# nyuolab/OmniBioTE

Hardware: AMD Instinct MI355X
Metric: MLM train tokens/sec, small (8L/1024d) ctx=1024 at 1/2/4/8 MI355X (higher is better)
Workload: dtype bf16

## Files before the change

omnibiote_amd/csrc/elementwise.hip:

```cpp
#include "common.h"
#include <stdlib.h>

namespace {

template <bool INVERSE>
__global__ __launch_bounds__(256) void rope_kernel(bf16* __restrict__ qkv, const float* __restrict__ cos_t,
                                                    const float* __restrict__ sin_t, int64_t rows, int64_t T, int C, int hs) {
    const int chunks_per_row = 2 * C / 8;
    const int64_t total = rows * chunks_per_row;
    for (int64_t i = (int64_t)blockIdx.x * blockDim.x + threadIdx.x; i < total; i += (int64_t)gridDim.x * blockDim.x) {
        const int64_t row = i / chunks_per_row;
        const int col = (int)(i % chunks_per_row) * 8;
        const int d = col % hs;
        const int64_t t = row % T;
        bf16* ptr = qkv + row * 3 * C + col;
        const bf16x8 v = *reinterpret_cast<const bf16x8*>(ptr);
        const f32x4 c = *reinterpret_cast<const f32x4*>(cos_t + t * (hs / 2) + d / 2);
        const f32x4 s = *reinterpret_cast<const f32x4*>(sin_t + t * (hs / 2) + d / 2);
        bf16x8 o;
#pragma unroll
        for (int j = 0; j < 4; ++j) {
            const float xe = bf2f(v[2 * j]), xo = bf2f(v[2 * j + 1]);
            const float sj = INVERSE ? -s[j] : s[j];
            o[2 * j] = f2bf(xe * c[j] - xo * sj);
            o[2 * j + 1] = f2bf(xe * sj + xo * c[j]);
        }
        *reinterpret_cast<bf16x8*>(ptr) = o;
    }
}

__device__ __forceinline__ int64_t clamp_tok(int64_t tok, int64_t vocab) { return tok < 0 ? 0 : (tok >= vocab ? vocab - 1 : tok); }

__global__ __launch_bounds__(256) void embed_fwd_kernel(const int64_t* __restrict__ idx, const bf16* __restrict__ wte,
                                                         bf16* __restrict__ out, int64_t rows, int cols, int64_t vocab, DropCfg dc) {
    const int cpr = cols / 8;
    const int64_t total = rows * cpr;
    for (int64_t i = (int64_t)blockIdx.x * blockDim.x + threadIdx.x; i < total; i += (int64_t)gridDim.x * blockDim.x) {
        const int64_t r = i / cpr;
        const int c = (int)(i % cpr) * 8;
        const int64_t tok = clamp_tok(idx[r], vocab);
        bf16x8 v = *reinterpret_cast<const bf16x8*>(wte + tok * cols + c);
        if (dc.thresh16) {
            const uint32_t rk = drop_rowkey((uint64_t)r, dc);
#pragma unroll
            for (int jj = 0; jj < 4; ++jj) {
                const uint32_t bits = drop_pair_bits(rk, (uint32_t)(c >> 1) + jj);
#pragma unroll
                for (int e = 0; e < 2; ++e) v[2 * jj + e] = drop_keep_bits(bits, (uint32_t)e, dc) ? f2bf(bf2f(v[2 * jj + e]) * dc.scale) : f2bf(0.f);
            }
        }
        *reinterpret_cast<bf16x8*>(out + r * cols + c) = v;
    }
}

__global__ __launch_bounds__(256) void dropout_kernel(const bf16* in, bf16* out, int64_t n8, int64_t cols, DropCfg dc) {
    for (int64_t i = (int64_t)blockIdx.x * blockDim.x + threadIdx.x; i < n8; i += (int64_t)gridDim.x * blockDim.x) {
        bf16x8 v = reinterpret_cast<const bf16x8*>(in)[i];
        const int64_t row = (i * 8) / cols;
        const uint32_t c = (uint32_t)((i * 8) - row * cols);
        const uint32_t rk = drop_rowkey((uint64_t)row, dc);
        for (int jj = 0; jj < 4; ++jj) {
            const uint32_t bits = drop_pair_bits(rk, (c >> 1) + jj);
#pragma unroll
            for (int e = 0; e < 2; ++e) v[2 * jj + e] = drop_keep_bits(bits, (uint32_t)e, dc) ? f2bf(bf2f(v[2 * jj + e]) * dc.scale) : f2bf(0.f);
        }
        reinterpret_cast<bf16x8*>(out)[i] = v;
    }
}

constexpr int EMB_CHUNK = 32;

template <bool ACC>
__device__ __forceinline__ void embed_store_row(bf16* dst, const float (&acc)[8]) {
    bf16x8 o;
#pragma unroll
    for (int j = 0; j < 8; ++j) o[j] = f2bf(acc[j]);
    if (ACC) {
        const bf16x8 old = *reinterpret_cast<const bf16x8*>(dst);
#pragma unroll
        for (int j = 0; j < 8; ++j) o[j] = f2bf(bf2f(old[j]) + bf2f(o[j]));
    }
    *reinterpret_cast<bf16x8*>(dst) = o;
}
template <bool ACC>
__device__ __forceinline__ void embed_store_row(float* dst, const float (&acc)[8]) {
    f32x4 lo = f32x4{acc[0], acc[1], acc[2], acc[3]}, hi = f32x4{acc[4], acc[5], acc[6], acc[7]};
    if (ACC) {
        lo += *reinterpret_cast<const f32x4*>(dst);
        hi += *reinterpret_cast<const f32x4*>(dst + 4);
    }
    *reinterpret_cast<f32x4*>(dst) = lo;
    *reinterpret_cast<f32x4*>(dst + 4) = hi;
}

template <bool ACC, class DST = bf16>
__global__ __launch_bounds__(128) void embed_bwd_chunk_kernel(const int64_t* __restrict__ idx, const int32_t* __restrict__ order,
                                                               const bf16* __restrict__ dout, DST* __restrict__ dwte,
                                                               float* __restrict__ slab, int64_t rows, int cols, int64_t vocab, DropCfg dc) {
    __shared__ int32_t s_row[EMB_CHUNK];
    __shared__ int64_t s_tok[EMB_CHUNK + 2];
    const int64_t c = blockIdx.x;
    const int64_t p0 = c * EMB_CHUNK;
    const int n = (int)((rows - p0) < EMB_CHUNK ? (rows - p0) : EMB_CHUNK);
    if (threadIdx.x < n) {
        const int32_t r = order[p0 + threadIdx.x];
        s_row[threadIdx.x] = r;
        s_tok[threadIdx.x + 1] = clamp_tok(idx[r], vocab);
    }
    if (threadIdx.x == 64) s_tok[0] = p0 > 0 ? clamp_tok(idx[order[p0 - 1]], vocab) : -1;
    if (threadIdx.x == 65) s_tok[n + 1] = (p0 + n < rows) ? clamp_tok(idx[order[p0 + n]], vocab) : -1;
    __syncthreads();
    const bool left_open = s_tok[0] == s_tok[1];
    const bool right_open = s_tok[n + 1] == s_tok[n];
    for (int col = threadIdx.x * 8; col < cols; col += 128 * 8) {
        float acc[8];
#pragma unroll
        for (int j = 0; j < 8; ++j) acc[j] = 0.f;
        int seg_start = 0;
        for (int i = 0; i < n; ++i) {
            const bf16x8 v = *reinterpret_cast<const bf16x8*>(dout + (int64_t)s_row[i] * cols + col);
            if (dc.thresh16) {
                const uint32_t rk = drop_rowkey((uint64_t)s_row[i], dc);
                for (int jj = 0; jj < 4; ++jj) {
                    const uint32_t bits = drop_pair_bits(rk, (uint32_t)(col >> 1) + jj);
#pragma unroll
                    for (int e = 0; e < 2; ++e)
                        if (drop_keep_bits(bits, (uint32_t)e, dc)) acc[2 * jj + e] += bf2f(f2bf(bf2f(v[2 * jj + e]) * dc.scale));
                }
            } else {
#pragma unroll
                for (int j = 0; j < 8; ++j) acc[j] += bf2f(v[j]);
            }
            const bool seg_end = (i == n - 1) || (s_tok[i + 2] != s_tok[i + 1]);
            if (seg_end) {
                const bool is_first = seg_start == 0, is_last = i == n - 1;
                if ((is_first && left_open) || (is_last && right_open)) {
                    float* dst = slab + ((c * 2 + (is_first ? 0 : 1)) * cols + col);
                    *reinterpret_cast<f32x4*>(dst) = f32x4{acc[0], acc[1], acc[2], acc[3]};
                    *reinterpret_cast<f32x4*>(dst + 4) = f32x4{acc[4], acc[5], acc[6], acc[7]};
                } else {
                    embed_store_row<ACC>(dwte + s_tok[i + 1] * cols + col, acc);
                }
#pragma unroll
                for (int j = 0; j < 8; ++j) acc[j] = 0.f;
                seg_start = i + 1;
            }
        }
    }
}

template <bool ACC, class DST = bf16>
__global__ __launch_bounds__(128) void embed_bwd_span_kernel(const int64_t* __restrict__ idx, const int32_t* __restrict__ order,
                                                              DST* __restrict__ dwte, const float* __restrict__ slab,
                                                              int64_t rows, int cols, int64_t nchunks, int64_t vocab) {
    const int64_t c = blockIdx.x;
    const int64_t p0 = c * EMB_CHUNK;
    const int64_t p1 = (p0 + EMB_CHUNK < rows) ? p0 + EMB_CHUNK : rows;
    const int64_t first = clamp_tok(idx[order[p0]], vocab), last = clamp_tok(idx[order[p1 - 1]], vocab);
    const bool single = first == last;
    const bool left_open = p0 > 0 && clamp_tok(idx[order[p0 - 1]], vocab) == first;
    const bool right_open = p1 < rows && clamp_tok(idx[order[p1]], vocab) == last;
    if (!right_open || (single && left_open)) return;
    const int slot0 = single ? 0 : 1;
    for (int col = threadIdx.x * 8; col < cols; col += 128 * 8) {
        float acc[8];
        const float* src = slab + ((c * 2 + slot0) * cols + col);
#pragma unroll
        for (int j = 0; j < 8; ++j) acc[j] = src[j];
        for (int64_t cc = c + 1; cc < nchunks; ++cc) {
            const int64_t q0 = cc * EMB_CHUNK;
            const int64_t q1 = (q0 + EMB_CHUNK < rows) ? q0 + EMB_CHUNK : rows;
            if (clamp_tok(idx[order[q0]], vocab) != last) break;
            const float* s2 = slab + ((cc * 2) * cols + col);
#pragma unroll
            for (int j = 0; j < 8; ++j) acc[j] += s2[j];
            if (clamp_tok(idx[order[q1 - 1]], vocab) != last) break;
        }
        embed_store_row<ACC>(dwte + last * cols + col, acc);
    }
}

__global__ __launch_bounds__(256) void acc32_add_kernel(float* __restrict__ acc32, const bf16* __restrict__ src, bf16* __restrict__ out,
                                                         int64_t n8, int mode) {
    for (int64_t i = (int64_t)blockIdx.x * 256 + threadIdx.x; i < n8; i += (int64_t)gridDim.x * 256) {
        float v[8];
        if (src) {
            const bf16x8 sv = *reinterpret_cast<const bf16x8*>(src + i * 8);
#pragma unroll
            for (int j = 0; j < 8; ++j) v[j] = bf2f(sv[j]);
        } else {
#pragma unroll
            for (int j = 0; j < 8; ++j) v[j] = 0.f;
        }
        if (mode != OBTE_ACC32_FIRST) {
            const f32x4 lo = *reinterpret_cast<const f32x4*>(acc32 + i * 8), hi = *reinterpret_cast<const f32x4*>(acc32 + i * 8 + 4);
#pragma unroll
            for (int j = 0; j < 4; ++j) { v[j] += lo[j]; v[4 + j] += hi[j]; }
        }
        if (src || mode == OBTE_ACC32_FIRST) {
            *reinterpret_cast<f32x4*>(acc32 + i * 8) = f32x4{v[0], v[1], v[2], v[3]};
            *reinterpret_cast<f32x4*>(acc32 + i * 8 + 4) = f32x4{v[4], v[5], v[6], v[7]};
        }
        if (mode == OBTE_ACC32_LAST) {
            bf16x8 o;
#pragma unroll
            for (int j = 0; j < 8; ++j) o[j] = f2bf(v[j]);
            *reinterpret_cast<bf16x8*>(out + i * 8) = o;
        }
    }
}

__global__ __launch_bounds__(256) void masked_ce_kernel(const bf16* __restrict__ logits, const int64_t* __restrict__ target,
                                                         const uint8_t* __restrict__ mlm_mask, const uint8_t* __restrict__ prev_mask,
                                                         const float* __restrict__ grad_scale, float row_scale,
                                                         float* __restrict__ row_loss, bf16* __restrict__ dlogits, int64_t vocab,
                                                         const int64_t* __restrict__ row_index, const float* __restrict__ row_scale_vec) {
    __shared__ float red[8];
    const int64_t r = blockIdx.x;
    const int64_t src = row_index ? row_index[r] : r;
    const int lane = threadIdx.x & 63, wave = threadIdx.x >> 6;
    bf16* drow = dlogits + r * vocab;
    if (!row_index && mlm_mask && !mlm_mask[r]) {
        if (threadIdx.x == 0 && row_loss) row_loss[r] = 0.f;
        if (prev_mask && !prev_mask[r]) return;
        const bf16x8 z = {};
        for (int64_t c = (int64_t)threadIdx.x * 8; c < vocab; c += 256 * 8) *reinterpret_cast<bf16x8*>(drow + c) = z;
        return;
    }
    const bf16* lrow = logits + src * vocab;
    float m = -INFINITY, l = 0.f;
    for (int64_t c = (int64_t)threadIdx.x * 8; c < vocab; c += 256 * 8) {
        const bf16x8 v = *reinterpret_cast<const bf16x8*>(lrow + c);
// ... 475 lines not shown
    const int lane = threadIdx.x & 63;
    const uint32_t rk = drop_rowkey((uint64_t)rows[i], cfg);
    for (int c = lane * 8; c < cols; c += 512) {
        bf16x8 v = *reinterpret_cast<const bf16x8*>(in + i * cols + c);
        bf16x8 a = {};
        if (aux) a = *reinterpret_cast<const bf16x8*>(aux + i * cols + c);
#pragma unroll
        for (int jj = 0; jj < 4; ++jj) {
            const uint32_t bits = drop_pair_bits(rk, ((uint32_t)c >> 1) + jj);
#pragma unroll
            for (int e = 0; e < 2; ++e) {
                const int j = 2 * jj + e;
                const float t = drop_keep_bits(bits, (uint32_t)e, cfg) ? bf2f(f2bf(bf2f(v[j]) * cfg.scale)) : 0.f;
                v[j] = aux ? f2bf(bf2f(a[j]) + t) : f2bf(t);
            }
        }
        *reinterpret_cast<bf16x8*>(out + i * cols + c) = v;
    }
}

extern "C" int obte_dropout_bf16(const obte_bf16* in, obte_bf16* out, int64_t n, int64_t cols, float p, uint64_t seed, int32_t site,
                                 obte_stream s) {
    OBTE_REQUIRE_ALIGNED("obte_dropout_bf16", in, "in", 16);
    OBTE_REQUIRE_ALIGNED("obte_dropout_bf16", out, "out", 16);
    OBTE_REQUIRE(in && out && n > 0 && n % 8 == 0, "obte_dropout_bf16: null pointer or n not a positive multiple of 8");
    OBTE_REQUIRE(cols > 0 && cols % 8 == 0 && n % cols == 0 && cols < (1ll << 32), "obte_dropout_bf16: cols must be a multiple of 8 that divides n");
    if (check_p("obte_dropout_bf16", p)) return OBTE_EINVAL;
    hipLaunchKernelGGL(dropout_kernel, dim3(stream_grid(n / 8, 256)), dim3(256), 0, (hipStream_t)s, (const bf16*)in, (bf16*)out, n / 8,
                       cols, make_drop(p, seed, (uint32_t)site));
    OBTE_CHECK_LAUNCH("obte_dropout_bf16");
    return OBTE_OK;
}

extern "C" int64_t obte_embedding_bwd_ws_bytes(int64_t rows, int cols) {
    return cdiv64(rows, EMB_CHUNK) * 2 * (int64_t)cols * (int64_t)sizeof(float);
}

extern "C" int obte_embedding_bwd_dropout(const int64_t* idx, const int32_t* order, const obte_bf16* dout, obte_bf16* dwte,
                                          void* ws, int64_t rows, int cols, int64_t vocab, int accumulate, float p, uint64_t seed,
                                          obte_stream s) {
    OBTE_REQUIRE(idx && order && dout && dwte && ws, "obte_embedding_bwd: null pointer");
    OBTE_REQUIRE_ALIGNED("obte_embedding_bwd", dout, "dout", 16);
    OBTE_REQUIRE_ALIGNED("obte_embedding_bwd", dwte, "dwte", 16);
    OBTE_REQUIRE_ALIGNED("obte_embedding_bwd", ws, "ws", 16);
    if (check_p("obte_embedding_bwd", p)) return OBTE_EINVAL;
    const DropCfg dc = make_drop(p, seed, OBTE_SITE_EMBED);
    OBTE_REQUIRE(rows > 0 && cols > 0 && cols % 8 == 0 && vocab > 0, "obte_embedding_bwd: bad shape");
    OBTE_REQUIRE(rows < (1ll << 31), "obte_embedding_bwd: too many rows");
    hipStream_t st = (hipStream_t)s;
    if (!accumulate && hipMemsetAsync(dwte, 0, (size_t)vocab * cols * sizeof(obte_bf16), st) != hipSuccess) {
        obte_set_error("obte_embedding_bwd: memset failed");
        return OBTE_ELAUNCH;
    }
    const int64_t nchunks = cdiv64(rows, EMB_CHUNK);
    if (accumulate)
        hipLaunchKernelGGL(embed_bwd_chunk_kernel<true>, dim3((unsigned)nchunks), dim3(128), 0, st, idx, order, (const bf16*)dout,
                           (bf16*)dwte, (float*)ws, rows, cols, vocab, dc);
    else
        hipLaunchKernelGGL(embed_bwd_chunk_kernel<false>, dim3((unsigned)nchunks), dim3(128), 0, st, idx, order, (const bf16*)dout,
                           (bf16*)dwte, (float*)ws, rows, cols, vocab, dc);
    OBTE_CHECK_LAUNCH("obte_embedding_bwd(chunk)");
    if (accumulate)
        hipLaunchKernelGGL(embed_bwd_span_kernel<true>, dim3((unsigned)nchunks), dim3(128), 0, st, idx, order, (bf16*)dwte,
                           (const float*)ws, rows, cols, nchunks, vocab);
    else
        hipLaunchKernelGGL(embed_bwd_span_kernel<false>, dim3((unsigned)nchunks), dim3(128), 0, st, idx, order, (bf16*)dwte,
                           (const float*)ws, rows, cols, nchunks, vocab);
    OBTE_CHECK_LAUNCH("obte_embedding_bwd(span)");
    return OBTE_OK;
}

extern "C" int obte_acc32_add_bf16(float* acc32, const obte_bf16* src, obte_bf16* out, int64_t n, int mode, obte_stream s) {
    OBTE_REQUIRE_ALIGNED("obte_acc32_add_bf16", acc32, "acc32", 16);
    OBTE_REQUIRE_ALIGNED("obte_acc32_add_bf16", src, "src", 16);
    OBTE_REQUIRE_ALIGNED("obte_acc32_add_bf16", out, "out", 16);
    OBTE_REQUIRE(acc32 && n > 0 && n % 8 == 0, "obte_acc32_add_bf16: null buffer or n not a positive multiple of 8");
    OBTE_REQUIRE(mode >= OBTE_ACC32_FIRST && mode <= OBTE_ACC32_LAST && (mode != OBTE_ACC32_LAST || out), "obte_acc32_add_bf16: bad mode, or LAST without out");
    if (!src && mode == OBTE_ACC32_MORE) return OBTE_OK;
    hipLaunchKernelGGL(acc32_add_kernel, dim3(stream_grid(n / 8, 256)), dim3(256), 0, (hipStream_t)s, acc32, (const bf16*)src, (bf16*)out, n / 8, mode);
    OBTE_CHECK_LAUNCH("obte_acc32_add_bf16");
    return OBTE_OK;
}

extern "C" int obte_embedding_bwd_acc32(const int64_t* idx, const int32_t* order, const obte_bf16* dout, float* acc32, obte_bf16* dwte,
                                        void* ws, int64_t rows, int cols, int64_t vocab, int mode, float p, uint64_t seed, obte_stream s) {
    OBTE_REQUIRE(idx && order && dout && acc32 && ws, "obte_embedding_bwd_acc32: null pointer");
    OBTE_REQUIRE_ALIGNED("obte_embedding_bwd_acc32", dout, "dout", 16);
    OBTE_REQUIRE_ALIGNED("obte_embedding_bwd_acc32", acc32, "acc32", 16);
    OBTE_REQUIRE_ALIGNED("obte_embedding_bwd_acc32", dwte, "dwte", 16);
    OBTE_REQUIRE_ALIGNED("obte_embedding_bwd_acc32", ws, "ws", 16);
    OBTE_REQUIRE(mode >= OBTE_ACC32_FIRST && mode <= OBTE_ACC32_LAST && (mode != OBTE_ACC32_LAST || dwte), "obte_embedding_bwd_acc32: bad mode, or LAST without dwte");
    if (check_p("obte_embedding_bwd_acc32", p)) return OBTE_EINVAL;
    const DropCfg dc = make_drop(p, seed, OBTE_SITE_EMBED);
    OBTE_REQUIRE(rows > 0 && cols > 0 && cols % 8 == 0 && vocab > 0, "obte_embedding_bwd_acc32: bad shape");
    OBTE_REQUIRE(rows < (1ll << 31), "obte_embedding_bwd_acc32: too many rows");
    hipStream_t st = (hipStream_t)s;
    const bool first = mode == OBTE_ACC32_FIRST;
    if (first && hipMemsetAsync(acc32, 0, (size_t)vocab * cols * sizeof(float), st) != hipSuccess) {
        obte_set_error("obte_embedding_bwd_acc32: memset failed");
        return OBTE_ELAUNCH;
    }
    const int64_t nchunks = cdiv64(rows, EMB_CHUNK);
    if (first)
        hipLaunchKernelGGL((embed_bwd_chunk_kernel<false, float>), dim3((unsigned)nchunks), dim3(128), 0, st, idx, order, (const bf16*)dout, acc32, (float*)ws,
                           rows, cols, vocab, dc);
    else
        hipLaunchKernelGGL((embed_bwd_chunk_kernel<true, float>), dim3((unsigned)nchunks), dim3(128), 0, st, idx, order, (const bf16*)dout, acc32, (float*)ws,
                           rows, cols, vocab, dc);
    OBTE_CHECK_LAUNCH("obte_embedding_bwd_acc32(chunk)");
    if (first)
        hipLaunchKernelGGL((embed_bwd_span_kernel<false, float>), dim3((unsigned)nchunks), dim3(128), 0, st, idx, order, acc32, (const float*)ws, rows, cols,
                           nchunks, vocab);
    else
        hipLaunchKernelGGL((embed_bwd_span_kernel<true, float>), dim3((unsigned)nchunks), dim3(128), 0, st, idx, order, acc32, (const float*)ws, rows, cols,
                           nchunks, vocab);
    OBTE_CHECK_LAUNCH("obte_embedding_bwd_acc32(span)");
    if (mode == OBTE_ACC32_LAST) return obte_acc32_add_bf16(acc32, nullptr, dwte, vocab * (int64_t)cols, OBTE_ACC32_LAST, s);
    return OBTE_OK;
}

extern "C" int obte_embedding_bwd_acc(const int64_t* idx, const int32_t* order, const obte_bf16* dout, obte_bf16* dwte,
                                      void* ws, int64_t rows, int cols, int64_t vocab, int accumulate, obte_stream s) {
    return obte_embedding_bwd_dropout(idx, order, dout, dwte, ws, rows, cols, vocab, accumulate, 0.f, 0, s);
}

extern "C" int obte_embedding_bwd(const int64_t* idx, const int32_t* order, const obte_bf16* dout, obte_bf16* dwte,
                                  void* ws, int64_t rows, int cols, int64_t vocab, obte_stream s) {
    return obte_embedding_bwd_dropout(idx, order, dout, dwte, ws, rows, cols, vocab, 0, 0.f, 0, s);
}

extern "C" int obte_masked_ce_fwd_bwd_reuse(const obte_bf16* logits, const int64_t* target, const uint8_t* mlm_mask,
                                            const uint8_t* prev_mask, const float* grad_scale, float row_scale, float* row_loss,
                                            obte_bf16* dlogits, int64_t rows, int64_t vocab, obte_stream s) {
    OBTE_REQUIRE(logits && target && mlm_mask && grad_scale && dlogits, "obte_masked_ce_fwd_bwd: null pointer");
    OBTE_REQUIRE_ALIGNED("obte_masked_ce_fwd_bwd", logits, "logits", 16);
    OBTE_REQUIRE_ALIGNED("obte_masked_ce_fwd_bwd", dlogits, "dlogits", 16);
    OBTE_REQUIRE(rows > 0 && rows < (1ll << 31) && vocab > 0 && vocab % 8 == 0, "obte_masked_ce_fwd_bwd: vocab must be a multiple of 8");
    hipLaunchKernelGGL(masked_ce_kernel, dim3((unsigned)rows), dim3(256), 0, (hipStream_t)s, (const bf16*)logits, target, mlm_mask,
                       prev_mask, grad_scale, row_scale, row_loss, (bf16*)dlogits, vocab, (const int64_t*)nullptr, (const float*)nullptr);
    OBTE_CHECK_LAUNCH("obte_masked_ce_fwd_bwd");
    return OBTE_OK;
}

namespace {
__global__ __launch_bounds__(256) void rows_copy_kernel(const bf16* __restrict__ src, const int64_t* __restrict__ rows, bf16* __restrict__ dst,
                                                         int64_t n_rows, int64_t total_rows, int cols, int scatter) {
    const int wave = threadIdx.x >> 6, lane = threadIdx.x & 63;
    const int64_t i = (int64_t)blockIdx.x * 4 + wave;
    if (i >= n_rows) return;
    int64_t r = rows[i];
    r = r < 0 ? 0 : (r >= total_rows ? total_rows - 1 : r);
    const bf16* s = src + (scatter ? i : r) * cols;
    bf16* d = dst + (scatter ? r : i) * cols;
    for (int c = lane * 8; c < cols; c += 64 * 8) *reinterpret_cast<bf16x8*>(d + c) = *reinterpret_cast<const bf16x8*>(s + c);
}
}
extern "C" int obte_rows_gather_bf16(const obte_bf16* src, const int64_t* rows, obte_bf16* dst, int64_t n_rows, int64_t total_rows, int32_t cols, obte_stream s) {
    OBTE_REQUIRE(src && rows && dst, "obte_rows_gather_bf16: null pointer");
    OBTE_REQUIRE_ALIGNED("obte_rows_gather_bf16", src, "src", 16);
    OBTE_REQUIRE_ALIGNED("obte_rows_gather_bf16", dst, "dst", 16);
    OBTE_REQUIRE(n_rows > 0 && total_rows > 0 && cols > 0 && cols % 8 == 0, "obte_rows_gather_bf16: need n_rows, total_rows > 0 and cols %% 8 == 0");
    hipLaunchKernelGGL(rows_copy_kernel, dim3((unsigned)cdiv64(n_rows, 4)), dim3(256), 0, (hipStream_t)s, (const bf16*)src, rows, (bf16*)dst, n_rows, total_rows, cols, 0);
    OBTE_CHECK_LAUNCH("obte_rows_gather_bf16");
    return OBTE_OK;
}
extern "C" int obte_rows_scatter_bf16(const obte_bf16* src, const int64_t* rows, obte_bf16* dst, int64_t n_rows, int64_t total_rows, int32_t cols, obte_stream s) {
    OBTE_REQUIRE(src && rows && dst, "obte_rows_scatter_bf16: null pointer");
    OBTE_REQUIRE_ALIGNED("obte_rows_scatter_bf16", src, "src", 16);
    OBTE_REQUIRE_ALIGNED("obte_rows_scatter_bf16", dst, "dst", 16);
// ... 252 lines not shown
```

Measured before the change: 1.298 million.

## Prefetch rows and precompute segment kinds in embedding backward kernels

The chunk kernel now handles two chunks per 256-thread block and precomputes each row's segment-end kind in shared memory. It double-buffers batches of dout rows and old dwte rows so global loads are issued ahead of the accumulation. The span kernel finds the run length of matching chunks with a wavefront ballot, splits columns across a second grid dimension, and batches slab loads. The aim is to hide memory latency in the serial per-row accumulation, at the cost of more registers and speculative loads of dwte rows that may never be written.

New measurement: 1.300 million, median of 4. No clear change (+0.1%).

```diff
diff --git a/omnibiote_amd/csrc/elementwise.hip b/omnibiote_amd/csrc/elementwise.hip
--- a/omnibiote_amd/csrc/elementwise.hip
+++ b/omnibiote_amd/csrc/elementwise.hip
@@ -69,90 +69,133 @@
 }
 
 constexpr int EMB_CHUNK = 32;
+constexpr int EMB_AHEAD = 8;
+constexpr int EMB_SLAB_AHEAD = 16;
+
+template <class DST> struct EmbRow;
+template <> struct EmbRow<bf16> { bf16x8 v; };
+template <> struct EmbRow<float> { f32x4 lo, hi; };
+__device__ __forceinline__ EmbRow<bf16> embed_load_row(const bf16* src) { return EmbRow<bf16>{*reinterpret_cast<const bf16x8*>(src)}; }
+__device__ __forceinline__ EmbRow<float> embed_load_row(const float* src) {
+    return EmbRow<float>{*reinterpret_cast<const f32x4*>(src), *reinterpret_cast<const f32x4*>(src + 4)};
+}
 
 template <bool ACC>
-__device__ __forceinline__ void embed_store_row(bf16* dst, const float (&acc)[8]) {
+__device__ __forceinline__ void embed_store_row(bf16* dst, const float (&acc)[8], const EmbRow<bf16>& old) {
     bf16x8 o;
 #pragma unroll
     for (int j = 0; j < 8; ++j) o[j] = f2bf(acc[j]);
     if (ACC) {
-        const bf16x8 old = *reinterpret_cast<const bf16x8*>(dst);
-#pragma unroll
-        for (int j = 0; j < 8; ++j) o[j] = f2bf(bf2f(old[j]) + bf2f(o[j]));
+#pragma unroll
+        for (int j = 0; j < 8; ++j) o[j] = f2bf(bf2f(old.v[j]) + bf2f(o[j]));
     }
     *reinterpret_cast<bf16x8*>(dst) = o;
 }
 template <bool ACC>
-__device__ __forceinline__ void embed_store_row(float* dst, const float (&acc)[8]) {
+__device__ __forceinline__ void embed_store_row(float* dst, const float (&acc)[8], const EmbRow<float>& old) {
     f32x4 lo = f32x4{acc[0], acc[1], acc[2], acc[3]}, hi = f32x4{acc[4], acc[5], acc[6], acc[7]};
     if (ACC) {
-        lo += *reinterpret_cast<const f32x4*>(dst);
-        hi += *reinterpret_cast<const f32x4*>(dst + 4);
+        lo += old.lo;
+        hi += old.hi;
     }
     *reinterpret_cast<f32x4*>(dst) = lo;
     *reinterpret_cast<f32x4*>(dst + 4) = hi;
 }
 
 template <bool ACC, class DST = bf16>
-__global__ __launch_bounds__(128) void embed_bwd_chunk_kernel(const int64_t* __restrict__ idx, const int32_t* __restrict__ order,
+__global__ __launch_bounds__(256) void embed_bwd_chunk_kernel(const int64_t* __restrict__ idx, const int32_t* __restrict__ order,
                                                                const bf16* __restrict__ dout, DST* __restrict__ dwte,
                                                                float* __restrict__ slab, int64_t rows, int cols, int64_t vocab, DropCfg dc) {
-    __shared__ int32_t s_row[EMB_CHUNK];
-    __shared__ int64_t s_tok[EMB_CHUNK + 2];
-    const int64_t c = blockIdx.x;
+    __shared__ int32_t s_row_[2][EMB_CHUNK];
+    __shared__ int64_t s_tok_[2][EMB_CHUNK + 2];
+    __shared__ int32_t s_kind_[2][EMB_CHUNK];
+    const int sub = threadIdx.x >> 7, tid = threadIdx.x & 127;
+    int32_t* const s_row = s_row_[sub];
+    int64_t* const s_tok = s_tok_[sub];
+    int32_t* const s_kind = s_kind_[sub];
+    const int64_t c = (int64_t)blockIdx.x * 2 + sub;
     const int64_t p0 = c * EMB_CHUNK;
-    const int n = (int)((rows - p0) < EMB_CHUNK ? (rows - p0) : EMB_CHUNK);
-    if (threadIdx.x < n) {
-        const int32_t r = order[p0 + threadIdx.x];
-        s_row[threadIdx.x] = r;
-        s_tok[threadIdx.x + 1] = clamp_tok(idx[r], vocab);
-    }
-    if (threadIdx.x == 64) s_tok[0] = p0 > 0 ? clamp_tok(idx[order[p0 - 1]], vocab) : -1;
-    if (threadIdx.x == 65) s_tok[n + 1] = (p0 + n < rows) ? clamp_tok(idx[order[p0 + n]], vocab) : -1;
+    const int n = p0 < rows ? (int)((rows - p0) < EMB_CHUNK ? (rows - p0) : EMB_CHUNK) : 0;
+    if (tid < EMB_CHUNK && n > 0) {
+        const int32_t r = order[p0 + (tid < n ? tid : n - 1)];
+        s_row[tid] = r;
+        if (tid < n) s_tok[tid + 1] = clamp_tok(idx[r], vocab);
+    }
+    if (tid == 64 && n > 0) s_tok[0] = p0 > 0 ? clamp_tok(idx[order[p0 - 1]], vocab) : -1;
+    if (tid == 65 && n > 0) s_tok[n + 1] = (p0 + n < rows) ? clamp_tok(idx[order[p0 + n]], vocab) : -1;
     __syncthreads();
-    const bool left_open = s_tok[0] == s_tok[1];
-    const bool right_open = s_tok[n + 1] == s_tok[n];
-    for (int col = threadIdx.x * 8; col < cols; col += 128 * 8) {
+    if (tid < EMB_CHUNK && n > 0) {
+        const int i = tid < n ? tid : n - 1;
+        const bool seg_end = (i == n - 1) || (s_tok[i + 2] != s_tok[i + 1]);
+        bool is_first = true;
+        for (int j = 0; j < i; ++j) is_first = is_first && s_tok[j + 2] == s_tok[j + 1];
+        const bool is_last = i == n - 1;
+        const bool left_open = s_tok[0] == s_tok[1], right_open = s_tok[n + 1] == s_tok[n];
+        const bool to_slab = (is_first && left_open) || (is_last && right_open);
+        s_kind[tid] = (tid < n && seg_end) ? (to_slab ? (is_first ? 2 : 3) : 1) : 0;
+    }
+    __syncthreads();
+    if (n == 0) return;
+    const int64_t tok_n = s_tok[n];
+    for (int col = tid * 8; col < cols; col += 128 * 8) {
+        bf16x8 v[2][EMB_AHEAD];
+        EmbRow<DST> old[2][EMB_AHEAD];
+        auto request = [&](int b, bf16x8 (&vb)[EMB_AHEAD], EmbRow<DST> (&ob)[EMB_AHEAD]) {
+#pragma unroll
+            for (int k = 0; k < EMB_AHEAD; ++k) {
+                const int i = b * EMB_AHEAD + k;
+                vb[k] = *reinterpret_cast<const bf16x8*>(dout + (int64_t)s_row[i] * cols + col);
+                if (ACC) ob[k] = embed_load_row(dwte + (i < n ? s_tok[i + 1] : tok_n) * cols + col);
+            }
+        };
         float acc[8];
 #pragma unroll
         for (int j = 0; j < 8; ++j) acc[j] = 0.f;
-        int seg_start = 0;
-        for (int i = 0; i < n; ++i) {
-            const bf16x8 v = *reinterpret_cast<const bf16x8*>(dout + (int64_t)s_row[i] * cols + col);
-            if (dc.thresh16) {
-                const uint32_t rk = drop_rowkey((uint64_t)s_row[i], dc);
-                for (int jj = 0; jj < 4; ++jj) {
-                    const uint32_t bits = drop_pair_bits(rk, (uint32_t)(col >> 1) + jj);
-#pragma unroll
-                    for (int e = 0; e < 2; ++e)
-                        if (drop_keep_bits(bits, (uint32_t)e, dc)) acc[2 * jj + e] += bf2f(f2bf(bf2f(v[2 * jj + e]) * dc.scale));
+        auto add_batch = [&](int b, const bf16x8 (&vb)[EMB_AHEAD], const EmbRow<DST> (&ob)[EMB_AHEAD]) {
+#pragma unroll
+            for (int k = 0; k < EMB_AHEAD; ++k) {
+                const int i = b * EMB_AHEAD + k;
+                if (i >= n) break;
+                if (dc.thresh16) {
+                    const uint32_t rk = drop_rowkey((uint64_t)s_row[i], dc);
+                    for (int jj = 0; jj < 4; ++jj) {
+                        const uint32_t bits = drop_pair_bits(rk, (uint32_t)(col >> 1) + jj);
+#pragma unroll
+                        for (int e = 0; e < 2; ++e)
+                            if (drop_keep_bits(bits, (uint32_t)e, dc)) acc[2 * jj + e] += bf2f(f2bf(bf2f(vb[k][2 * jj + e]) * dc.scale));
+                    }
+                } else {
+#pragma unroll
+                    for (int j = 0; j < 8; ++j) acc[j] += bf2f(vb[k][j]);
                 }
-            } else {
-#pragma unroll
-                for (int j = 0; j < 8; ++j) acc[j] += bf2f(v[j]);
+                const int kind = s_kind[i];
+                if (kind) {
+                    if (kind >= 2) {
+                        float* dst = slab + ((c * 2 + (kind - 2)) * cols + col);
+                        *reinterpret_cast<f32x4*>(dst) = f32x4{acc[0], acc[1], acc[2], acc[3]};
+                        *reinterpret_cast<f32x4*>(dst + 4) = f32x4{acc[4], acc[5], acc[6], acc[7]};
+                    } else {
+                        embed_store_row<ACC>(dwte + s_tok[i + 1] * cols + col, acc, ob[k]);
+                    }
+#pragma unroll
+                    for (int j = 0; j < 8; ++j) acc[j] = 0.f;
+                }
             }
-            const bool seg_end = (i == n - 1) || (s_tok[i + 2] != s_tok[i + 1]);
-            if (seg_end) {
-                const bool is_first = seg_start == 0, is_last = i == n - 1;
-                if ((is_first && left_open) || (is_last && right_open)) {
-                    float* dst = slab + ((c * 2 + (is_first ? 0 : 1)) * cols + col);
-                    *reinterpret_cast<f32x4*>(dst) = f32x4{acc[0], acc[1], acc[2], acc[3]};
-                    *reinterpret_cast<f32x4*>(dst + 4) = f32x4{acc[4], acc[5], acc[6], acc[7]};
-                } else {
-                    embed_store_row<ACC>(dwte + s_tok[i + 1] * cols + col, acc);
-                }
-#pragma unroll
-                for (int j = 0; j < 8; ++j) acc[j] = 0.f;
-                seg_start = i + 1;
-            }
+        };
+        constexpr int NB = EMB_CHUNK / EMB_AHEAD;
+        request(0, v[0], old[0]);
+#pragma unroll
+        for (int b = 0; b < NB; ++b) {
+            if (b + 1 < NB && (b + 1) * EMB_AHEAD < n) request(b + 1, v[(b + 1) & 1], old[(b + 1) & 1]);
+            if (b * EMB_AHEAD < n) add_batch(b, v[b & 1], old[b & 1]);
         }
     }
 }
 
 template <bool ACC, class DST = bf16>
-__global__ __launch_bounds__(128) void embed_bwd_span_kernel(const int64_t* __restrict__ idx, const int32_t* __restrict__ order,
-                                                              DST* __restrict__ dwte, const float* __restrict__ slab,
-                                                              int64_t rows, int cols, int64_t nchunks, int64_t vocab) {
+__global__ __launch_bounds__(64) void embed_bwd_span_kernel(const int64_t* __restrict__ idx, const int32_t* __restrict__ order,
+                                                             DST* __restrict__ dwte, const float* __restrict__ slab,
+                                                             int64_t rows, int cols, int64_t nchunks, int64_t vocab) {
     const int64_t c = blockIdx.x;
     const int64_t p0 = c * EMB_CHUNK;
     const int64_t p1 = (p0 + EMB_CHUNK < rows) ? p0 + EMB_CHUNK : rows;
@@ -162,22 +205,41 @@
     const bool right_open = p1 < rows && clamp_tok(idx[order[p1]], vocab) == last;
     if (!right_open || (single && left_open)) return;
     const int slot0 = single ? 0 : 1;
-    for (int col = threadIdx.x * 8; col < cols; col += 128 * 8) {
-        float acc[8];
-        const float* src = slab + ((c * 2 + slot0) * cols + col);
-#pragma unroll
-        for (int j = 0; j < 8; ++j) acc[j] = src[j];
-        for (int64_t cc = c + 1; cc < nchunks; ++cc) {
-            const int64_t q0 = cc * EMB_CHUNK;
-            const int64_t q1 = (q0 + EMB_CHUNK < rows) ? q0 + EMB_CHUNK : rows;
-            if (clamp_tok(idx[order[q0]], vocab) != last) break;
+    int64_t n_more = 0;
+    for (int64_t base = c + 1; base < nchunks; base += 64) {
+        const int64_t cc = base + threadIdx.x;
+        const bool mine = cc < nchunks && clamp_tok(idx[order[cc * EMB_CHUNK]], vocab) == last;
+        const unsigned long long others = ~__ballot(mine);
+        const int lead = others ? __builtin_ctzll(others) : 64;
+        n_more += lead;
+        if (lead < 64) break;
+    }
+    const int col = (int)blockIdx.y * 512 + (int)threadIdx.x * 8;
+    if (col >= cols || n_more == 0) return;
+    EmbRow<DST> old{};
+    if (ACC) old = embed_load_row(dwte + last * cols + col);
+    float acc[8];
+    const float* src = slab + ((c * 2 + slot0) * cols + col);
+#pragma unroll
+    for (int j = 0; j < 8; ++j) acc[j] = src[j];
+    for (int64_t k0 = 0; k0 < n_more; k0 += EMB_SLAB_AHEAD) {
+        f32x4 lo[EMB_SLAB_AHEAD], hi[EMB_SLAB_AHEAD];
+#pragma unroll
+        for (int k = 0; k < EMB_SLAB_AHEAD; ++k) {
+            const int64_t cc = c + 1 + (k0 + k < n_more ? k0 + k : n_more - 1);
             const float* s2 = slab + ((cc * 2) * cols + col);
-#pragma unroll
-            for (int j = 0; j < 8; ++j) acc[j] += s2[j];
-            if (clamp_tok(idx[order[q1 - 1]], vocab) != last) break;
-        }
-        embed_store_row<ACC>(dwte + last * cols + col, acc);
-    }
+            lo[k] = *reinterpret_cast<const f32x4*>(s2);
+            hi[k] = *reinterpret_cast<const f32x4*>(s2 + 4);
+        }
+#pragma unroll
+        for (int k = 0; k < EMB_SLAB_AHEAD; ++k) {
+            if (k0 + k < n_more) {
+#pragma unroll
+                for (int j = 0; j < 4; ++j) { acc[j] += lo[k][j]; acc[4 + j] += hi[k][j]; }
+            }
+        }
+    }
+    embed_store_row<ACC>(dwte + last * cols + col, acc, old);
 }
 
 __global__ __launch_bounds__(256) void acc32_add_kernel(float* __restrict__ acc32, const bf16* __restrict__ src, bf16* __restrict__ out,
@@ -761,17 +823,17 @@
     }
     const int64_t nchunks = cdiv64(rows, EMB_CHUNK);
     if (accumulate)
-        hipLaunchKernelGGL(embed_bwd_chunk_kernel<true>, dim3((unsigned)nchunks), dim3(128), 0, st, idx, order, (const bf16*)dout,
+        hipLaunchKernelGGL(embed_bwd_chunk_kernel<true>, dim3((unsigned)cdiv64(nchunks, 2)), dim3(256), 0, st, idx, order, (const bf16*)dout,
                            (bf16*)dwte, (float*)ws, rows, cols, vocab, dc);
     else
-        hipLaunchKernelGGL(embed_bwd_chunk_kernel<false>, dim3((unsigned)nchunks), dim3(128), 0, st, idx, order, (const bf16*)dout,
+        hipLaunchKernelGGL(embed_bwd_chunk_kernel<false>, dim3((unsigned)cdiv64(nchunks, 2)), dim3(256), 0, st, idx, order, (const bf16*)dout,
                            (bf16*)dwte, (float*)ws, rows, cols, vocab, dc);
     OBTE_CHECK_LAUNCH("obte_embedding_bwd(chunk)");
     if (accumulate)
-        hipLaunchKernelGGL(embed_bwd_span_kernel<true>, dim3((unsigned)nchunks), dim3(128), 0, st, idx, order, (bf16*)dwte,
+        hipLaunchKernelGGL(embed_bwd_span_kernel<true>, dim3((unsigned)nchunks, (unsigned)cdiv64(cols, 512)), dim3(64), 0, st, idx, order, (bf16*)dwte,
                            (const float*)ws, rows, cols, nchunks, vocab);
     else
-        hipLaunchKernelGGL(embed_bwd_span_kernel<false>, dim3((unsigned)nchunks), dim3(128), 0, st, idx, order, (bf16*)dwte,
+        hipLaunchKernelGGL(embed_bwd_span_kernel<false>, dim3((unsigned)nchunks, (unsigned)cdiv64(cols, 512)), dim3(64), 0, st, idx, order, (bf16*)dwte,
                            (const float*)ws, rows, cols, nchunks, vocab);
     OBTE_CHECK_LAUNCH("obte_embedding_bwd(span)");
     return OBTE_OK;
@@ -809,17 +871,17 @@
     }
     const int64_t nchunks = cdiv64(rows, EMB_CHUNK);
     if (first)
-        hipLaunchKernelGGL((embed_bwd_chunk_kernel<false, float>), dim3((unsigned)nchunks), dim3(128), 0, st, idx, order, (const bf16*)dout, acc32, (float*)ws,
+        hipLaunchKernelGGL((embed_bwd_chunk_kernel<false, float>), dim3((unsigned)cdiv64(nchunks, 2)), dim3(256), 0, st, idx, order, (const bf16*)dout, acc32, (float*)ws,
                            rows, cols, vocab, dc);
     else
-        hipLaunchKernelGGL((embed_bwd_chunk_kernel<true, float>), dim3((unsigned)nchunks), dim3(128), 0, st, idx, order, (const bf16*)dout, acc32, (float*)ws,
+        hipLaunchKernelGGL((embed_bwd_chunk_kernel<true, float>), dim3((unsigned)cdiv64(nchunks, 2)), dim3(256), 0, st, idx, order, (const bf16*)dout, acc32, (float*)ws,
                            rows, cols, vocab, dc);
     OBTE_CHECK_LAUNCH("obte_embedding_bwd_acc32(chunk)");
     if (first)
-        hipLaunchKernelGGL((embed_bwd_span_kernel<false, float>), dim3((unsigned)nchunks), dim3(128), 0, st, idx, order, acc32, (const float*)ws, rows, cols,
+        hipLaunchKernelGGL((embed_bwd_span_kernel<false, float>), dim3((unsigned)nchunks, (unsigned)cdiv64(cols, 512)), dim3(64), 0, st, idx, order, acc32, (const float*)ws, rows, cols,
                            nchunks, vocab);
     else
-        hipLaunchKernelGGL((embed_bwd_span_kernel<true, float>), dim3((unsigned)nchunks), dim3(128), 0, st, idx, order, acc32, (const float*)ws, rows, cols,
+        hipLaunchKernelGGL((embed_bwd_span_kernel<true, float>), dim3((unsigned)nchunks, (unsigned)cdiv64(cols, 512)), dim3(64), 0, st, idx, order, acc32, (const float*)ws, rows, cols,
                            nchunks, vocab);
     OBTE_CHECK_LAUNCH("obte_embedding_bwd_acc32(span)");
     if (mode == OBTE_ACC32_LAST) return obte_acc32_add_bf16(acc32, nullptr, dwte, vocab * (int64_t)cols, OBTE_ACC32_LAST, s);
```

## Restructure embedding backward kernels with batched prefetch and parallel span reduction

Applied to the files above, without the earlier changes.

The chunk kernel now precomputes segment-end kinds in LDS, packs several chunks per 256-thread block when cols is small, and software-pipelines the dout and old-dwte loads in batches of eight rows. The span kernel counts matching follow-on chunks with a block-wide vote, then parallelises over columns through a 2D grid with per-element batched loads. The aim is to hide memory latency and remove serial per-row dependence in the embedding gradient scatter. In exchange it adds register pressure and wider span launches, and the chunk kernel assumes a full chunk of rows, clamping out-of-range reads to the last row.

New measurement: 1.276 million before, 1.278 million after (median of 4 runs). Within noise of the previous version (+0.1%).

```diff
diff --git a/omnibiote_amd/csrc/elementwise.hip b/omnibiote_amd/csrc/elementwise.hip
--- a/omnibiote_amd/csrc/elementwise.hip
+++ b/omnibiote_amd/csrc/elementwise.hip
@@ -69,90 +69,157 @@
 }
 
 constexpr int EMB_CHUNK = 32;
+constexpr int EMB_THREADS = 256;
+constexpr int EMB_BATCH = 8;
+constexpr int EMB_MAX_CPW = 32;
+
+template <class DST> struct EmbOld;
+template <> struct EmbOld<bf16> { bf16x8 v; };
+template <> struct EmbOld<float> { f32x4 lo, hi; };
+__device__ __forceinline__ void embed_load_old(EmbOld<bf16>& o, const bf16* src) { o.v = *reinterpret_cast<const bf16x8*>(src); }
+__device__ __forceinline__ void embed_load_old(EmbOld<float>& o, const float* src) {
+    o.lo = *reinterpret_cast<const f32x4*>(src);
+    o.hi = *reinterpret_cast<const f32x4*>(src + 4);
+}
 
 template <bool ACC>
-__device__ __forceinline__ void embed_store_row(bf16* dst, const float (&acc)[8]) {
+__device__ __forceinline__ void embed_store_row(bf16* dst, const float (&acc)[8], const EmbOld<bf16>& old) {
     bf16x8 o;
 #pragma unroll
     for (int j = 0; j < 8; ++j) o[j] = f2bf(acc[j]);
     if (ACC) {
-        const bf16x8 old = *reinterpret_cast<const bf16x8*>(dst);
-#pragma unroll
-        for (int j = 0; j < 8; ++j) o[j] = f2bf(bf2f(old[j]) + bf2f(o[j]));
+#pragma unroll
+        for (int j = 0; j < 8; ++j) o[j] = f2bf(bf2f(old.v[j]) + bf2f(o[j]));
     }
     *reinterpret_cast<bf16x8*>(dst) = o;
 }
 template <bool ACC>
-__device__ __forceinline__ void embed_store_row(float* dst, const float (&acc)[8]) {
+__device__ __forceinline__ void embed_store_row(float* dst, const float (&acc)[8], const EmbOld<float>& old) {
     f32x4 lo = f32x4{acc[0], acc[1], acc[2], acc[3]}, hi = f32x4{acc[4], acc[5], acc[6], acc[7]};
     if (ACC) {
-        lo += *reinterpret_cast<const f32x4*>(dst);
-        hi += *reinterpret_cast<const f32x4*>(dst + 4);
+        lo += old.lo;
+        hi += old.hi;
     }
     *reinterpret_cast<f32x4*>(dst) = lo;
     *reinterpret_cast<f32x4*>(dst + 4) = hi;
 }
+template <bool ACC>
+__device__ __forceinline__ void embed_store_elem(bf16* dst, float acc) {
+    bf16 o = f2bf(acc);
+    if (ACC) o = f2bf(bf2f(*dst) + bf2f(o));
+    *dst = o;
+}
+template <bool ACC>
+__device__ __forceinline__ void embed_store_elem(float* dst, float acc) {
+    if (ACC) acc += *dst;
+    *dst = acc;
+}
+
+struct EmbChunkLds {
+    int64_t tok[EMB_CHUNK + 2];
+    int32_t row[EMB_CHUNK];
+    uint8_t kind[EMB_CHUNK];
+};
+enum : uint8_t { EMB_NONE = 0, EMB_ROW = 1, EMB_SLOT0 = 2, EMB_SLOT1 = 3 };
 
 template <bool ACC, class DST = bf16>
-__global__ __launch_bounds__(128) void embed_bwd_chunk_kernel(const int64_t* __restrict__ idx, const int32_t* __restrict__ order,
-                                                               const bf16* __restrict__ dout, DST* __restrict__ dwte,
-                                                               float* __restrict__ slab, int64_t rows, int cols, int64_t vocab, DropCfg dc) {
-    __shared__ int32_t s_row[EMB_CHUNK];
-    __shared__ int64_t s_tok[EMB_CHUNK + 2];
-    const int64_t c = blockIdx.x;
-    const int64_t p0 = c * EMB_CHUNK;
-    const int n = (int)((rows - p0) < EMB_CHUNK ? (rows - p0) : EMB_CHUNK);
-    if (threadIdx.x < n) {
-        const int32_t r = order[p0 + threadIdx.x];
-        s_row[threadIdx.x] = r;
-        s_tok[threadIdx.x + 1] = clamp_tok(idx[r], vocab);
-    }
-    if (threadIdx.x == 64) s_tok[0] = p0 > 0 ? clamp_tok(idx[order[p0 - 1]], vocab) : -1;
-    if (threadIdx.x == 65) s_tok[n + 1] = (p0 + n < rows) ? clamp_tok(idx[order[p0 + n]], vocab) : -1;
+__global__ __launch_bounds__(EMB_THREADS) void embed_bwd_chunk_kernel(const int64_t* __restrict__ idx, const int32_t* __restrict__ order,
+                                                                       const bf16* __restrict__ dout, DST* __restrict__ dwte,
+                                                                       float* __restrict__ slab, int64_t rows, int cols, int64_t vocab, DropCfg dc,
+                                                                       int cpw) {
+    extern __shared__ __attribute__((aligned(16))) char emb_smem[];
+    EmbChunkLds* lds = reinterpret_cast<EmbChunkLds*>(emb_smem);
+    const int64_t c0 = (int64_t)blockIdx.x * cpw;
+    for (int e = threadIdx.x; e < cpw * (EMB_CHUNK + 2); e += EMB_THREADS) {
+        const int lc = e / (EMB_CHUNK + 2), k = e % (EMB_CHUNK + 2);
+        const int64_t p0 = (c0 + lc) * EMB_CHUNK;
+        if (p0 >= rows) continue;
+        const int64_t pos = p0 - 1 + k;
+        lds[lc].tok[k] = (pos >= 0 && pos < rows) ? clamp_tok(idx[order[pos]], vocab) : -1;
+        if (k >= 1 && k <= EMB_CHUNK) lds[lc].row[k - 1] = order[pos < rows ? pos : rows - 1];
+    }
     __syncthreads();
-    const bool left_open = s_tok[0] == s_tok[1];
-    const bool right_open = s_tok[n + 1] == s_tok[n];
-    for (int col = threadIdx.x * 8; col < cols; col += 128 * 8) {
+    for (int e = threadIdx.x; e < cpw * EMB_CHUNK; e += EMB_THREADS) {
+        const int lc = e / EMB_CHUNK, i = e % EMB_CHUNK;
+        const int64_t p0 = (c0 + lc) * EMB_CHUNK;
+        if (p0 >= rows) continue;
+        const int n = (int)((rows - p0) < EMB_CHUNK ? (rows - p0) : EMB_CHUNK);
+        const int64_t* t = lds[lc].tok;
+        uint8_t kind = EMB_NONE;
+        if (i < n && (i == n - 1 || t[i + 2] != t[i + 1])) {
+            const bool is_first = t[i + 1] == t[1], is_last = i == n - 1;
+            const bool left_open = t[0] == t[1], right_open = t[n + 1] == t[n];
+            kind = !((is_first && left_open) || (is_last && right_open)) ? EMB_ROW : is_first ? EMB_SLOT0 : EMB_SLOT1;
+        }
+        lds[lc].kind[i] = kind;
+    }
+    __syncthreads();
+    const int ppc = cols / 8;
+    const int tpc = ppc < EMB_THREADS ? ppc : EMB_THREADS;
+    const int lc = threadIdx.x / tpc;
+    const int64_t c = c0 + lc;
+    if (lc >= cpw || c * EMB_CHUNK >= rows) return;
+    const EmbChunkLds& L = lds[lc];
+    for (int col = ((int)threadIdx.x - lc * tpc) * 8; col < cols; col += tpc * 8) {
         float acc[8];
 #pragma unroll
         for (int j = 0; j < 8; ++j) acc[j] = 0.f;
-        int seg_start = 0;
-        for (int i = 0; i < n; ++i) {
-            const bf16x8 v = *reinterpret_cast<const bf16x8*>(dout + (int64_t)s_row[i] * cols + col);
-            if (dc.thresh16) {
-                const uint32_t rk = drop_rowkey((uint64_t)s_row[i], dc);
-                for (int jj = 0; jj < 4; ++jj) {
-                    const uint32_t bits = drop_pair_bits(rk, (uint32_t)(col >> 1) + jj);
-#pragma unroll
-                    for (int e = 0; e < 2; ++e)
-                        if (drop_keep_bits(bits, (uint32_t)e, dc)) acc[2 * jj + e] += bf2f(f2bf(bf2f(v[2 * jj + e]) * dc.scale));
+        auto load = [&](bf16x8 (&v)[EMB_BATCH], EmbOld<DST> (&o)[EMB_BATCH], int b) {
+#pragma unroll
+            for (int j = 0; j < EMB_BATCH; ++j) {
+                const int i = b + j;
+                v[j] = *reinterpret_cast<const bf16x8*>(dout + (int64_t)L.row[i] * cols + col);
+                if (ACC && L.kind[i] == EMB_ROW) embed_load_old(o[j], dwte + L.tok[i + 1] * cols + col);
+            }
+        };
+        auto add = [&](const bf16x8 (&v)[EMB_BATCH], const EmbOld<DST> (&o)[EMB_BATCH], int b) {
+#pragma unroll
+            for (int j = 0; j < EMB_BATCH; ++j) {
+                const int i = b + j;
+                if (dc.thresh16) {
+                    const uint32_t rk = drop_rowkey((uint64_t)L.row[i], dc);
+#pragma unroll
+                    for (int jj = 0; jj < 4; ++jj) {
+                        const uint32_t bits = drop_pair_bits(rk, (uint32_t)(col >> 1) + jj);
+#pragma unroll
+                        for (int e = 0; e < 2; ++e)
+                            if (drop_keep_bits(bits, (uint32_t)e, dc)) acc[2 * jj + e] += bf2f(f2bf(bf2f(v[j][2 * jj + e]) * dc.scale));
+                    }
+                } else {
+#pragma unroll
+                    for (int e = 0; e < 8; ++e) acc[e] += bf2f(v[j][e]);
                 }
-            } else {
-#pragma unroll
-                for (int j = 0; j < 8; ++j) acc[j] += bf2f(v[j]);
+                const int kind = L.kind[i];
+                if (kind != EMB_NONE) {
+                    if (kind == EMB_ROW) {
+                        embed_store_row<ACC>(dwte + L.tok[i + 1] * cols + col, acc, o[j]);
+                    } else {
+                        float* dst = slab + ((c * 2 + (kind - EMB_SLOT0)) * cols + col);
+                        *reinterpret_cast<f32x4*>(dst) = f32x4{acc[0], acc[1], acc[2], acc[3]};
+                        *reinterpret_cast<f32x4*>(dst + 4) = f32x4{acc[4], acc[5], acc[6], acc[7]};
+                    }
+#pragma unroll
+                    for (int e = 0; e < 8; ++e) acc[e] = 0.f;
+                }
             }
-            const bool seg_end = (i == n - 1) || (s_tok[i + 2] != s_tok[i + 1]);
-            if (seg_end) {
-                const bool is_first = seg_start == 0, is_last = i == n - 1;
-                if ((is_first && left_open) || (is_last && right_open)) {
-                    float* dst = slab + ((c * 2 + (is_first ? 0 : 1)) * cols + col);
-                    *reinterpret_cast<f32x4*>(dst) = f32x4{acc[0], acc[1], acc[2], acc[3]};
-                    *reinterpret_cast<f32x4*>(dst + 4) = f32x4{acc[4], acc[5], acc[6], acc[7]};
-                } else {
-                    embed_store_row<ACC>(dwte + s_tok[i + 1] * cols + col, acc);
-                }
-#pragma unroll
-                for (int j = 0; j < 8; ++j) acc[j] = 0.f;
-                seg_start = i + 1;
-            }
+        };
+        bf16x8 va[EMB_BATCH], vb[EMB_BATCH];
+        EmbOld<DST> oa[EMB_BATCH], ob[EMB_BATCH];
+        load(va, oa, 0);
+#pragma unroll 1
+        for (int b = 0; b < EMB_CHUNK; b += 2 * EMB_BATCH) {
+            load(vb, ob, b + EMB_BATCH);
+            add(va, oa, b);
+            if (b + 2 * EMB_BATCH < EMB_CHUNK) load(va, oa, b + 2 * EMB_BATCH);
+            add(vb, ob, b + EMB_BATCH);
         }
     }
 }
 
 template <bool ACC, class DST = bf16>
-__global__ __launch_bounds__(128) void embed_bwd_span_kernel(const int64_t* __restrict__ idx, const int32_t* __restrict__ order,
-                                                              DST* __restrict__ dwte, const float* __restrict__ slab,
-                                                              int64_t rows, int cols, int64_t nchunks, int64_t vocab) {
+__global__ __launch_bounds__(EMB_THREADS) void embed_bwd_span_kernel(const int64_t* __restrict__ idx, const int32_t* __restrict__ order,
+                                                                      DST* __restrict__ dwte, const float* __restrict__ slab,
+                                                                      int64_t rows, int cols, int64_t nchunks, int64_t vocab) {
     const int64_t c = blockIdx.x;
     const int64_t p0 = c * EMB_CHUNK;
     const int64_t p1 = (p0 + EMB_CHUNK < rows) ? p0 + EMB_CHUNK : rows;
@@ -162,22 +229,53 @@
     const bool right_open = p1 < rows && clamp_tok(idx[order[p1]], vocab) == last;
     if (!right_open || (single && left_open)) return;
     const int slot0 = single ? 0 : 1;
-    for (int col = threadIdx.x * 8; col < cols; col += 128 * 8) {
-        float acc[8];
-        const float* src = slab + ((c * 2 + slot0) * cols + col);
-#pragma unroll
-        for (int j = 0; j < 8; ++j) acc[j] = src[j];
-        for (int64_t cc = c + 1; cc < nchunks; ++cc) {
-            const int64_t q0 = cc * EMB_CHUNK;
-            const int64_t q1 = (q0 + EMB_CHUNK < rows) ? q0 + EMB_CHUNK : rows;
-            if (clamp_tok(idx[order[q0]], vocab) != last) break;
-            const float* s2 = slab + ((cc * 2) * cols + col);
-#pragma unroll
-            for (int j = 0; j < 8; ++j) acc[j] += s2[j];
-            if (clamp_tok(idx[order[q1 - 1]], vocab) != last) break;
-        }
-        embed_store_row<ACC>(dwte + last * cols + col, acc);
-    }
+    int64_t m = 0;
+    for (int64_t base = c + 1; base < nchunks; base += EMB_THREADS) {
+        const int64_t cc = base + threadIdx.x;
+        const bool match = cc < nchunks && clamp_tok(idx[order[cc * EMB_CHUNK]], vocab) == last;
+        const int cnt = __syncthreads_count(match);
+        m += cnt;
+        if (cnt < EMB_THREADS) break;
+    }
+    const int col = (int)blockIdx.y * EMB_THREADS + (int)threadIdx.x;
+    if (col >= cols) return;
+    const int64_t stride = 2 * (int64_t)cols;
+    const float* src = slab + ((c + 1) * stride + col);
+    auto load = [&](float (&v)[EMB_BATCH], int64_t k) {
+#pragma unroll
+        for (int j = 0; j < EMB_BATCH; ++j) v[j] = (k + j < m) ? src[(k + j) * stride] : 0.f;
+    };
+    float acc = slab[(c * 2 + slot0) * cols + col];
+    auto add = [&](const float (&v)[EMB_BATCH], int64_t k) {
+#pragma unroll
+        for (int j = 0; j < EMB_BATCH; ++j)
+            if (k + j < m) acc += v[j];
+    };
+    float va[EMB_BATCH], vb[EMB_BATCH];
+    load(va, 0);
+#pragma unroll 1
+    for (int64_t k = 0; k < m; k += 2 * EMB_BATCH) {
+        load(vb, k + EMB_BATCH);
+        add(va, k);
+        load(va, k + 2 * EMB_BATCH);
+        add(vb, k + EMB_BATCH);
+    }
+    embed_store_elem<ACC>(dwte + last * cols + col, acc);
+}
+
+template <bool ACC, class DST>
+static int embed_bwd_launch(const char* who_chunk, const char* who_span, const int64_t* idx, const int32_t* order, const bf16* dout, DST* dwte,
+                            float* ws, int64_t rows, int cols, int64_t vocab, const DropCfg& dc, hipStream_t st) {
+    const int64_t nchunks = cdiv64(rows, EMB_CHUNK);
+    const int ppc = cols / 8;
+    const int cpw = ppc >= EMB_THREADS ? 1 : (EMB_THREADS / ppc < EMB_MAX_CPW ? EMB_THREADS / ppc : EMB_MAX_CPW);
+    hipLaunchKernelGGL((embed_bwd_chunk_kernel<ACC, DST>), dim3((unsigned)cdiv64(nchunks, cpw)), dim3(EMB_THREADS), cpw * sizeof(EmbChunkLds), st,
+                       idx, order, dout, dwte, ws, rows, cols, vocab, dc, cpw);
+    OBTE_CHECK_LAUNCH(who_chunk);
+    hipLaunchKernelGGL((embed_bwd_span_kernel<ACC, DST>), dim3((unsigned)nchunks, (unsigned)cdiv64(cols, EMB_THREADS)), dim3(EMB_THREADS), 0, st,
+                       idx, order, dwte, (const float*)ws, rows, cols, nchunks, vocab);
+    OBTE_CHECK_LAUNCH(who_span);
+    return OBTE_OK;
 }
 
 __global__ __launch_bounds__(256) void acc32_add_kernel(float* __restrict__ acc32, const bf16* __restrict__ src, bf16* __restrict__ out,
@@ -759,22 +857,11 @@
         obte_set_error("obte_embedding_bwd: memset failed");
         return OBTE_ELAUNCH;
     }
-    const int64_t nchunks = cdiv64(rows, EMB_CHUNK);
     if (accumulate)
-        hipLaunchKernelGGL(embed_bwd_chunk_kernel<true>, dim3((unsigned)nchunks), dim3(128), 0, st, idx, order, (const bf16*)dout,
-                           (bf16*)dwte, (float*)ws, rows, cols, vocab, dc);
-    else
-        hipLaunchKernelGGL(embed_bwd_chunk_kernel<false>, dim3((unsigned)nchunks), dim3(128), 0, st, idx, order, (const bf16*)dout,
-                           (bf16*)dwte, (float*)ws, rows, cols, vocab, dc);
-    OBTE_CHECK_LAUNCH("obte_embedding_bwd(chunk)");
-    if (accumulate)
-        hipLaunchKernelGGL(embed_bwd_span_kernel<true>, dim3((unsigned)nchunks), dim3(128), 0, st, idx, order, (bf16*)dwte,
-                           (const float*)ws, rows, cols, nchunks, vocab);
-    else
-        hipLaunchKernelGGL(embed_bwd_span_kernel<false>, dim3((unsigned)nchunks), dim3(128), 0, st, idx, order, (bf16*)dwte,
-                           (const float*)ws, rows, cols, nchunks, vocab);
-    OBTE_CHECK_LAUNCH("obte_embedding_bwd(span)");
-    return OBTE_OK;
+        return embed_bwd_launch<true, bf16>("obte_embedding_bwd(chunk)", "obte_embedding_bwd(span)", idx, order, (const bf16*)dout, (bf16*)dwte, (float*)ws,
+                                            rows, cols, vocab, dc, st);
+    return embed_bwd_launch<false, bf16>("obte_embedding_bwd(chunk)", "obte_embedding_bwd(span)", idx, order, (const bf16*)dout, (bf16*)dwte, (float*)ws,
+                                         rows, cols, vocab, dc, st);
 }
 
 extern "C" int obte_acc32_add_bf16(float* acc32, const obte_bf16* src, obte_bf16* out, int64_t n, int mode, obte_stream s) {
@@ -807,21 +894,11 @@
         obte_set_error("obte_embedding_bwd_acc32: memset failed");
         return OBTE_ELAUNCH;
     }
-    const int64_t nchunks = cdiv64(rows, EMB_CHUNK);
-    if (first)
-        hipLaunchKernelGGL((embed_bwd_chunk_kernel<false, float>), dim3((unsigned)nchunks), dim3(128), 0, st, idx, order, (const bf16*)dout, acc32, (float*)ws,
-                           rows, cols, vocab, dc);
-    else
-        hipLaunchKernelGGL((embed_bwd_chunk_kernel<true, float>), dim3((unsigned)nchunks), dim3(128), 0, st, idx, order, (const bf16*)dout, acc32, (float*)ws,
-                           rows, cols, vocab, dc);
-    OBTE_CHECK_LAUNCH("obte_embedding_bwd_acc32(chunk)");
-    if (first)
-        hipLaunchKernelGGL((embed_bwd_span_kernel<false, float>), dim3((unsigned)nchunks), dim3(128), 0, st, idx, order, acc32, (const float*)ws, rows, cols,
-                           nchunks, vocab);
-    else
-        hipLaunchKernelGGL((embed_bwd_span_kernel<true, float>), dim3((unsigned)nchunks), dim3(128), 0, st, idx, order, acc32, (const float*)ws, rows, cols,
-                           nchunks, vocab);
-    OBTE_CHECK_LAUNCH("obte_embedding_bwd_acc32(span)");
+    const int rc = first ? embed_bwd_launch<false, float>("obte_embedding_bwd_acc32(chunk)", "obte_embedding_bwd_acc32(span)", idx, order, (const bf16*)dout,
+                                                          acc32, (float*)ws, rows, cols, vocab, dc, st)
+                         : embed_bwd_launch<true, float>("obte_embedding_bwd_acc32(chunk)", "obte_embedding_bwd_acc32(span)", idx, order, (const bf16*)dout,
+                                                         acc32, (float*)ws, rows, cols, vocab, dc, st);
+    if (rc != OBTE_OK) return rc;
     if (mode == OBTE_ACC32_LAST) return obte_acc32_add_bf16(acc32, nullptr, dwte, vocab * (int64_t)cols, OBTE_ACC32_LAST, s);
     return OBTE_OK;
 }
```
